# jbush001/RustNetworkStack

Measured on AMD Instinct MI355X. Metric: GiB/s device-resident Internet checksum, 1500B-packet batches, 1/2/4/8 GPUs, higher is better.
Workload: dtype u8

## Files before the change

rustnetworkstack_amd/csrc/k_packed.hip:

```cpp
#include "rns_launch.hpp"

#ifndef RNS_ROWS_DEEP_FROM
#define RNS_ROWS_DEEP_FROM 1024u
#endif
#ifndef RNS_TX_ROWS_DEEP_FROM
#define RNS_TX_ROWS_DEEP_FROM 1024u
#endif
#ifndef RNS_RX_ROWS_D
#define RNS_RX_ROWS_D 8
#endif

namespace rns {

constexpr bool kStreamNT = RNS_STREAM_NT != 0;

template <class Kernel>
static int launch_rows(const CsumArgs &a, uint32_t deep_from, hipStream_t st, Kernel kernel)
{
    return with_flags(
        [&](auto deep, auto buf) {
            return launch(kernel(std::integral_constant<int, deep() ? 16 : 8>{}, buf), dim3(waves64(a.n)), dim3(64), 0,
                          st, a);
        },
        a.len_hint >= deep_from, buf_ok(a));
}

int launch_stream_rx(const CsumArgs &a, hipStream_t st)
{
    return with_flags(
        [&](auto ack, auto buf) {
            if constexpr (ack())
                return launch(csum_stream_kernel<kStreamNT, buf()>, dim3(waves64(a.n)), dim3(64), 0, st, a);
            else
                return launch(csum_rows_rx_kernel<kStreamNT, buf(), RNS_RX_ROWS_D>, dim3(waves64(a.n)), dim3(64), 0, st,
                              a);
        },
        a.arena_bytes / a.n <= 128, buf_ok(a));
}

int dispatch_packed(const CsumArgs &a, const Shape &sh, hipStream_t st)
{
    const bool tiny = (sh.variant & ~16u) == 3u && sh.G == 4u && sh.U == 1u;
    if (a.align_mask >= 15u && !tiny)
        return launch_rows(a, RNS_ROWS_DEEP_FROM, st,
                           [](auto D, auto buf) { return csum_rows_kernel<kStreamNT, buf(), D()>; });
    const bool mixed = (sh.variant & 4u) != 0;
    if (!mixed && !tiny)
        return RNS_E_INVALID;
    const uint64_t batches = waves64(a.n);
    const uint64_t wpb = (mixed ? kMixedBlock<false> : kBlock) / 64;
    uint64_t blocks = (batches + wpb - 1) / wpb;
    if (sh.max_blocks != 0 && blocks > sh.max_blocks)
        blocks = sh.max_blocks;
    const dim3 grid(static_cast<uint32_t>(blocks)), block(mixed ? kMixedBlock<false> : kBlock);
    if (mixed)
        return with_flags(
            [&](auto nt, auto buf) {
                return launch(csum_mixed_kernel<false, nt(), buf(), false, false, false, true>, grid, block, 0, st, a);
            },
            (sh.variant & 2u) != 0, buf_ok(a));
    return with_flags(
        [&](auto buf, auto pf) {
            return launch(csum_rounds_kernel<4, 1, false, true, buf(), 1, true, pf()>, grid, block, 0, st, a);
        },
        buf_ok(a), (sh.variant & 16u) != 0);
}

int launch_fill_packed(const CsumArgs &a, hipStream_t st)
{
    return launch_rows(a, RNS_ROWS_DEEP_FROM, st,
                       [](auto D, auto buf) { return csum_rows_kernel<kStreamNT, buf(), D(), true>; });
}

int launch_tx_packed(const CsumArgs &a, hipStream_t st)
{
    return launch_rows(a, RNS_TX_ROWS_DEEP_FROM, st,
                       [](auto D, auto buf) { return csum_rows_tx_kernel<kStreamNT, buf(), D()>; });
}

int launch_strided_rx(const CsumArgs &a, hipStream_t st)
{
    constexpr int B = kStridedRxB;
    const dim3 grid(static_cast<uint32_t>((static_cast<uint64_t>(a.n) + 64 * B - 1) / (64 * B)));
    return with_flags([&](auto buf) { return launch(csum_strided_rx_kernel<buf(), B>, grid, dim3(64), 0, st, a); },
                      buf_ok(a));
}

}
```

rustnetworkstack_amd/csrc/rns_checksum.hip:

```cpp
#include <hip/hip_runtime.h>

#include <algorithm>
#include <cmath>
#include <cstdint>
#include <cstdio>

#include "rns_launch.hpp"

using namespace rns;

namespace {

__global__ __launch_bounds__(kBlock) void splitmix64_fill_kernel(uint8_t *buf, uint64_t nbytes, uint64_t seed)
{
    const uint64_t nwords = (nbytes + 7) / 8;
    const uint64_t stride = static_cast<uint64_t>(gridDim.x) * blockDim.x;
    for (uint64_t i = static_cast<uint64_t>(blockIdx.x) * blockDim.x + threadIdx.x; i < nwords; i += stride) {
        uint64_t z = seed + (i + 1) * 0x9E3779B97F4A7C15ull;
        z = (z ^ (z >> 30)) * 0xBF58476D1CE4E5B9ull;
        z = (z ^ (z >> 27)) * 0x94D049BB133111EBull;
        z = z ^ (z >> 31);
        if ((i + 1) * 8 <= nbytes) {
            reinterpret_cast<uint64_t *>(buf)[i] = z;
        } else {
// ... 69 lines not shown
}

void set_field(CsumArgs &a, const uint16_t *d_field, uint32_t field_off)
{
    a.field = d_field;
    a.field_off = field_off;
}

uint32_t be_sum(const uint8_t *p, int nbytes)
{
    uint32_t s = 0;
    for (int k = 0; k < nbytes; k += 2)
        s += static_cast<uint32_t>(p[k]) << 8 | p[k + 1];
    return s;
}

void set_rx(CsumArgs &a, uint8_t *d_status, uint16_t *d_l4_sum, const uint8_t *local_ipv4, const uint8_t *local_ipv6)
{
    a.status = d_status;
    a.l4_out = d_l4_sum;
    a.local4_sum = be_sum(local_ipv4, 4);
    a.local6_sum = be_sum(local_ipv6, 16);
}

bool rx_valid(const uint8_t *d_status, const uint8_t *local_ipv4, const uint8_t *local_ipv6)
{
    return d_status && local_ipv4 && local_ipv6;
}

void set_tx_status(CsumArgs &a, uint8_t *d_status) { a.status = d_status; }

uint32_t chain_pick_k(double mean)
{
    uint32_t K = 1;
    double best = -1.0;
    for (uint32_t k = 1; k <= kChainMaxK; ++k) {
        const double fr = k * mean, fill = fr > 0 ? fr / std::ceil(fr) : 1.0;
        if (fill > best + 0.02) {
            best = fill;
            K = k;
        }
    }
    return K;
}

double chain_mean(const CsumArgs &a) { return static_cast<double>(a.n_frags) / static_cast<double>(a.n); }

#ifndef RNS_CHAIN_NT_FROM
#define RNS_CHAIN_NT_FROM 384u
#endif
bool chain_nt_from_hint(uint32_t frag_len_hint) { return (frag_len_hint ? frag_len_hint : 512u) >= RNS_CHAIN_NT_FROM; }
bool chain_nt_from_arena(uint64_t arena_bytes, uint32_t n_frags, double mean)
{
    const double frag_est = mean > 0.5 ? static_cast<double>(arena_bytes) / n_frags * (mean - 0.5) / mean : 0.0;
    return n_frags == 0 || frag_est >= RNS_CHAIN_NT_FROM;
}

bool chain_deep(uint32_t K, double mean) { return K >= 3 || (K == 2 && mean >= 2.0); }

template <bool FILL>
int chain_launch(CsumArgs &a, uint32_t frag_len_hint, hipStream_t stream)
{
    const double mean = chain_mean(a);
    a.chain_k = chain_pick_k(mean);
    if ((a.flags & RNS_FLAG_CHAIN_TX_PACKED) && mean <= 1.0 + kRunFrags)
        return launch_txrows<FILL>(a, stream);
    const bool runs = kChainRuns && (a.flags & RNS_FLAG_CHAIN_RUNS) && buf_ok(a);
    return launch_chain<FILL>(a, a.chain_k, chain_nt_from_hint(frag_len_hint), runs, chain_deep(a.chain_k, mean), stream);
}

constexpr uint64_t kRxGridCap = 4096;
dim3 stash_grid(uint64_t n, uint64_t arena_bytes, bool tiny_cap)
{
    constexpr int BLK = kMixedBlock<true>;
    uint64_t blocks = (waves64(n) + BLK / 64 - 1) / (BLK / 64);
    const bool cap = tiny_cap && arena_bytes / n <= 128;
    if (cap && blocks > kRxGridCap)
        blocks = kRxGridCap;
    return dim3(static_cast<uint32_t>(blocks));
}

bool misaligned(const void *p, uintptr_t mask) { return (reinterpret_cast<uintptr_t>(p) & mask) != 0; }

bool pool_rx_valid(const uint8_t *d_pool, uint32_t buf_log2, uint32_t min_log2, const uint32_t *d_buf_idx, uint32_t n_frags,
                   const uint32_t *d_blk_first, const uint16_t *d_len16, uint32_t n_pkts, const uint8_t *local_ipv4,
                   const uint8_t *local_ipv6, const uint8_t *d_status)
{
    return d_pool && buf_log2 >= min_log2 && buf_log2 <= kPoolMaxLog2 && d_blk_first && d_len16 && (!n_frags || d_buf_idx) &&
           n_pkts <= RNS_CHAIN_MAX_PACKETS && !misaligned(d_pool, 15) && rx_valid(d_status, local_ipv4, local_ipv6);
}

int pool_rx_verify(PoolRx &rx, bool &nt, const uint8_t *d_pool, uint64_t pool_bytes, uint32_t buf_log2,
                   const uint32_t *d_buf_idx, uint32_t n_frags, const uint32_t *d_blk_first, const uint16_t *d_len16,
                   uint32_t n_pkts, const uint8_t *local_ipv4, const uint8_t *local_ipv6, uint8_t *d_status, uint16_t *d_l4_sum,
                   void *stream)
{
    RNS_TRY(rns_rx_verify_pool_dev(d_pool, pool_bytes, buf_log2, d_buf_idx, n_frags, d_blk_first, d_len16, n_pkts, local_ipv4,
                                   local_ipv6, d_status, d_l4_sum, stream));
    rx = PoolRx{d_pool, pool_bytes, d_buf_idx, d_blk_first, d_len16, d_status, n_pkts, n_frags, buf_log2};
    nt = chain_nt_from_arena(pool_bytes, n_frags, static_cast<double>(n_frags) / n_pkts);
    return RNS_OK;
}

bool pool_tx_valid(const uint8_t *d_tx_pool, const uint32_t *d_free, uint32_t n_free, uint32_t cap, const uint32_t *d_ip_id_add,
                   const uint32_t *d_tx_blk_first, const uint8_t *d_tx_head_len8, const uint16_t *d_tx_pay_len16,
                   const uint32_t *d_tx_src, const uint32_t *d_count)
{
    return d_tx_pool && d_count && (!n_free || d_free) && (!cap || (d_tx_blk_first && d_tx_head_len8 && d_tx_pay_len16)) &&
           !misaligned(d_tx_pool, 15) && !misaligned(d_free, 3) && !misaligned(d_ip_id_add, 3) &&
           !misaligned(d_tx_blk_first, 3) && !misaligned(d_tx_pay_len16, 1) && !misaligned(d_tx_src, 3) &&
           !misaligned(d_count, 3);
}

void set_pool_tx(PoolTx &tx, uint8_t *d_tx_pool, uint64_t tx_pool_bytes, uint32_t buf_log2, const uint32_t *d_free,
                 uint32_t n_free, uint32_t cap, uint16_t ip_id_base, const uint32_t *d_ip_id_add, uint32_t *d_tx_blk_first,
                 uint8_t *d_tx_head_len8, uint16_t *d_tx_pay_len16, uint32_t *d_tx_src, uint32_t *d_count)
{
    tx = PoolTx{d_tx_pool, tx_pool_bytes >> buf_log2, d_free, d_ip_id_add, d_tx_blk_first, d_tx_head_len8, d_tx_pay_len16,
                d_tx_src, d_count, n_free, cap, ip_id_base, buf_log2};
}

int count_only(uint32_t *d_count, size_t bytes, void *stream)
{
    if (!d_count || misaligned(d_count, 3))
        return RNS_E_INVALID;
    RNS_TRY(check_device());
    return launch_fill32(d_count, bytes / 4, 0u, static_cast<hipStream_t>(stream));
}

}

extern "C" {

int rns_csum_batch_dev_cfg(const uint8_t *d_arena, uint64_t arena_bytes, const uint64_t *d_off,
                           const uint32_t *d_len, const uint16_t *d_seed, uint16_t *d_out, uint32_t n,
                           uint32_t flags, uint32_t variant, uint32_t lanes_per_packet, uint32_t unroll,
                           uint32_t max_blocks, uint32_t *d_bad, void *stream)
{
    return entry(n, d_off && d_len && d_out, d_arena, arena_bytes, flags, stream, [&](CsumArgs &a, hipStream_t st) {
        set_explicit(a, d_off, d_len);
        set_results(a, d_seed, d_out, d_bad);
        return dispatch<false>(a, variant, lanes_per_packet, unroll, max_blocks, st);
    });
}

int rns_csum_batch_dev(const uint8_t *d_arena, uint64_t arena_bytes, const uint64_t *d_off,
                       const uint32_t *d_len, const uint16_t *d_seed, uint16_t *d_out, uint32_t n,
                       uint32_t flags, uint32_t len_hint, uint32_t *d_bad, void *stream)
{
    const Shape sh = pick_shape(len_hint);
    return rns_csum_batch_dev_cfg(d_arena, arena_bytes, d_off, d_len, d_seed, d_out, n, flags, sh.variant, sh.G,
                                  sh.U, sh.max_blocks, d_bad, stream);
}

int rns_csum_batch_dev_off32(const uint8_t *d_arena, uint64_t arena_bytes, const uint32_t *d_off32,
                             const uint32_t *d_len, const uint16_t *d_seed, uint16_t *d_out, uint32_t n,
                             uint32_t flags, uint32_t len_hint, uint32_t *d_bad, void *stream)
{
    return entry(n, d_off32 && d_len && d_out, d_arena, arena_bytes, flags, stream, [&](CsumArgs &a, hipStream_t st) {
        a.off32 = d_off32;
        a.len = d_len;
        set_results(a, d_seed, d_out, d_bad);
        const Shape sh = pick_shape(len_hint);
        return dispatch<false>(a, sh.variant, sh.G, sh.U, sh.max_blocks, st);
    });
}

int rns_csum_batch_packed_dev(const uint8_t *d_arena, uint64_t arena_bytes, const uint64_t *d_blk_off,
                              const uint16_t *d_len16, uint32_t align_log2, const uint16_t *d_seed, uint16_t *d_out,
                              uint32_t n, uint32_t flags, uint32_t len_hint, uint32_t *d_bad, void *stream)
{
    return entry(n, d_blk_off && d_len16 && d_out && packed_align(align_log2, 0), d_arena, arena_bytes, flags, stream,
                 [&](CsumArgs &a, hipStream_t st) {
                     set_packed(a, d_blk_off, d_len16, align_log2);
                     set_results(a, d_seed, d_out, d_bad);
                     a.len_hint = len_hint;
                     Shape sh = pick_shape(len_hint);
                     if ((sh.variant & 5u) == 0)
                         sh = Shape{6u, 0u, 0u, 0u};
                     return dispatch_packed(a, sh, st);
                 });
}

int rns_csum_batch_strided_dev(const uint8_t *d_arena, uint64_t arena_bytes, uint64_t first_off,
                               uint64_t stride, uint32_t len, const uint16_t *d_seed, uint16_t *d_out,
                               uint32_t n, uint32_t flags, uint32_t *d_bad, void *stream)
{
    return entry(n, d_out && strided_fits(first_off, stride, n), d_arena, arena_bytes, flags, stream,
                 [&](CsumArgs &a, hipStream_t st) {
                     set_strided(a, first_off, stride);
                     set_results(a, d_seed, d_out, d_bad);
                     a.fixed_len = len;
                     if (len != 0 && len <= 64 && ((first_off + a.base_adjust) & 15) == 0 && (stride & 15) == 0)
                         return launch_strided_tiny(a, st);
                     const Shape sh = pick_shape(len);
                     return dispatch<true>(a, sh.variant, sh.G, sh.U, sh.max_blocks, st);
                 });
}

int rns_csum_chain_dev(const uint8_t *d_arena, uint64_t arena_bytes, const uint64_t *d_frag_off,
                       const uint32_t *d_frag_len, uint32_t n_frags, const uint32_t *d_first,
                       const uint16_t *d_seed, uint16_t *d_out, uint32_t n_pkts, uint32_t flags,
                       uint32_t frag_len_hint, uint16_t *d_frag_sums, uint32_t *d_bad, void *stream)
{
    (void)d_frag_sums;
    return entry(n_pkts, d_out && chain_valid(d_frag_off, d_frag_len, d_first, n_frags, n_pkts), d_arena, arena_bytes,
                 flags, stream, [&](CsumArgs &a, hipStream_t st) {
                     set_chain(a, d_frag_off, d_frag_len, d_first, n_frags);
                     set_results(a, d_seed, d_out, d_bad);
                     return chain_launch<false>(a, frag_len_hint, st);
                 });
}

int rns_csum_chain_fill_dev(uint8_t *d_arena, uint64_t arena_bytes, const uint64_t *d_frag_off,
                            const uint32_t *d_frag_len, uint32_t n_frags, const uint32_t *d_first,
                            const uint16_t *d_seed, const uint16_t *d_field, uint32_t field_off, uint16_t *d_out,
                            uint32_t n_pkts, uint32_t flags, uint32_t frag_len_hint, uint32_t *d_bad, void *stream)
{
    return entry(n_pkts, chain_valid(d_frag_off, d_frag_len, d_first, n_frags, n_pkts), d_arena, arena_bytes, flags,
                 stream, [&](CsumArgs &a, hipStream_t st) {
                     set_chain(a, d_frag_off, d_frag_len, d_first, n_frags);
                     set_results(a, d_seed, d_out, d_bad);
                     set_field(a, d_field, field_off);
                     return chain_launch<true>(a, frag_len_hint, st);
                 });
}

int rns_csum_fill_dev(uint8_t *d_arena, uint64_t arena_bytes, const uint64_t *d_off, const uint32_t *d_len,
                      const uint16_t *d_seed, const uint16_t *d_field, uint32_t field_off, uint16_t *d_out,
                      uint32_t n, uint32_t flags, uint32_t *d_bad, void *stream)
{
    return entry(n, d_off && d_len, d_arena, arena_bytes, flags, stream, [&](CsumArgs &a, hipStream_t st) {
        set_explicit(a, d_off, d_len);
        set_results(a, d_seed, d_out, d_bad);
        set_field(a, d_field, field_off);
        return launch_fill(a, stash_grid(n, arena_bytes, false), st);
    });
}

int rns_csum_fill_packed_dev(uint8_t *d_arena, uint64_t arena_bytes, const uint64_t *d_blk_off, const uint16_t *d_len16,
                             uint32_t align_log2, const uint16_t *d_seed, const uint16_t *d_field, uint32_t field_off,
                             uint16_t *d_out, uint32_t n, uint32_t flags, uint32_t len_hint, uint32_t *d_bad,
                             void *stream)
{
    return entry(n, d_blk_off && d_len16 && packed_align(align_log2, 4), d_arena, arena_bytes, flags, stream,
                 [&](CsumArgs &a, hipStream_t st) {
                     set_packed(a, d_blk_off, d_len16, align_log2);
                     set_results(a, d_seed, d_out, d_bad);
                     set_field(a, d_field, field_off);
                     a.len_hint = len_hint;
                     return launch_fill_packed(a, st);
                 });
}

int rns_rx_verify_dev(const uint8_t *d_arena, uint64_t arena_bytes, const uint64_t *d_off, const uint32_t *d_len,
                      uint32_t n, const uint8_t *local_ipv4, const uint8_t *local_ipv6, uint8_t *d_status,
                      uint16_t *d_l4_sum, void *stream)
{
    return entry(n, d_off && d_len && rx_valid(d_status, local_ipv4, local_ipv6), d_arena, arena_bytes,
                 RNS_FLAG_COMPLEMENT, stream, [&](CsumArgs &a, hipStream_t st) {
                     set_explicit(a, d_off, d_len);
                     set_rx(a, d_status, d_l4_sum, local_ipv4, local_ipv6);
                     return launch_rx(a, stash_grid(n, arena_bytes, true), st);
                 });
}

int rns_rx_verify_packed_dev(const uint8_t *d_arena, uint64_t arena_bytes, const uint64_t *d_blk_off,
                             const uint16_t *d_len16, uint32_t align_log2, uint32_t n, const uint8_t *local_ipv4,
                             const uint8_t *local_ipv6, uint8_t *d_status, uint16_t *d_l4_sum, void *stream)
{
    return entry(n, d_blk_off && d_len16 && rx_valid(d_status, local_ipv4, local_ipv6) && packed_align(align_log2, 4),
                 d_arena, arena_bytes, RNS_FLAG_COMPLEMENT, stream, [&](CsumArgs &a, hipStream_t st) {
                     set_packed(a, d_blk_off, d_len16, align_log2);
                     set_rx(a, d_status, d_l4_sum, local_ipv4, local_ipv6);
                     return launch_stream_rx(a, st);
                 });
}

int rns_rx_verify_strided_dev(const uint8_t *d_arena, uint64_t arena_bytes, uint64_t first_off, uint64_t stride,
                              const uint16_t *d_len16, uint32_t n, const uint8_t *local_ipv4, const uint8_t *local_ipv6,
                              uint8_t *d_status, uint16_t *d_l4_sum, void *stream)
{
    return entry(n, d_len16 && rx_valid(d_status, local_ipv4, local_ipv6) && strided_fits(first_off, stride, n), d_arena,
                 arena_bytes, RNS_FLAG_COMPLEMENT, stream, [&](CsumArgs &a, hipStream_t st) {
                     a.len16 = d_len16;
                     set_strided(a, first_off, stride);
                     set_rx(a, d_status, d_l4_sum, local_ipv4, local_ipv6);
                     return launch_strided_rx(a, st);
                 });
}

int rns_rx_verify_chain_dev(const uint8_t *d_arena, uint64_t arena_bytes, const uint64_t *d_frag_off,
                            const uint32_t *d_frag_len, uint32_t n_frags, const uint32_t *d_first, uint32_t n_pkts,
                            const uint8_t *local_ipv4, const uint8_t *local_ipv6, uint8_t *d_status, uint16_t *d_l4_sum,
                            void *stream)
{
    return entry(n_pkts,
                 chain_valid(d_frag_off, d_frag_len, d_first, n_frags, n_pkts) &&
                     rx_valid(d_status, local_ipv4, local_ipv6),
                 d_arena, arena_bytes, RNS_FLAG_COMPLEMENT, stream, [&](CsumArgs &a, hipStream_t st) {
                     set_chain(a, d_frag_off, d_frag_len, d_first, n_frags);
                     set_rx(a, d_status, d_l4_sum, local_ipv4, local_ipv6);
                     const double mean = chain_mean(a);
                     a.chain_k = chain_pick_k(mean);
                     return launch_rx_chain(a, a.chain_k, chain_nt_from_arena(arena_bytes, n_frags, mean), st);
                 });
}

int rns_rx_verify_pool_dev(const uint8_t *d_pool, uint64_t pool_bytes, uint32_t buf_log2, const uint32_t *d_buf_idx,
                           uint32_t n_frags, const uint32_t *d_blk_first, const uint16_t *d_len16, uint32_t n_pkts,
                           const uint8_t *local_ipv4, const uint8_t *local_ipv6, uint8_t *d_status, uint16_t *d_l4_sum,
                           void *stream)
{
    return entry(n_pkts,
                 pool_rx_valid(d_pool, buf_log2, kPoolMinLog2, d_buf_idx, n_frags, d_blk_first, d_len16, n_pkts, local_ipv4,
                               local_ipv6, d_status),
                 d_pool, pool_bytes, RNS_FLAG_COMPLEMENT, stream, [&](CsumArgs &a, hipStream_t st) {
                     a.off32 = d_buf_idx;
                     a.n_frags = n_frags;
                     a.first = d_blk_first;
                     a.len16 = d_len16;
                     a.align_mask = (1u << buf_log2) - 1u;
                     set_rx(a, d_status, d_l4_sum, local_ipv4, local_ipv6);
                     const double mean = chain_mean(a);
                     a.chain_k = chain_pick_k(mean);
                     return launch_rx_pool(a, a.chain_k, chain_nt_from_arena(pool_bytes, n_frags, mean), st);
                 });
}

int rns_rx_tcp_place_pool_dev(const uint8_t *d_pool, uint64_t pool_bytes, uint32_t buf_log2, const uint32_t *d_buf_idx,
                              uint32_t n_frags, const uint32_t *d_blk_first, const uint16_t *d_len16, uint32_t n_pkts,
                              const uint8_t *local_ipv4, const uint8_t *local_ipv6, const uint8_t *d_tbl,
                              uint64_t tbl_bytes, const uint32_t *d_next_seq, const uint64_t *d_win_off,
                              const uint32_t *d_win_len, uint32_t n_flows, uint8_t *d_stream, uint64_t stream_bytes,
                              uint8_t *d_status, uint16_t *d_l4_sum, rns_rx_tcp_meta *d_meta, void *stream)
{
    static_assert(sizeof(rns_rx_tcp_meta) == 24 && sizeof(rns_rx_flow_key) == kFlowSlotBytes - 8, "rns_k_pool_place.hpp");
    if (n_pkts == 0)
        return RNS_OK;
    const uint64_t slots = flow_slots(n_flows);
    if (!pool_rx_valid(d_pool, buf_log2, kPlaceMinLog2, d_buf_idx, n_frags, d_blk_first, d_len16, n_pkts, local_ipv4,
                       local_ipv6, d_status) ||
        !d_meta || misaligned(d_meta, 3) || !d_next_seq || !d_win_off || !d_win_len || !d_stream ||
        (n_flows && (!d_tbl || misaligned(d_tbl, 3) || tbl_bytes < slots * kFlowSlotBytes)))
        return RNS_E_INVALID;
    PoolRx rx;
// ... 382 lines not shown
                     set_tx_status(a, d_status);
                     return launch_txrows<false, true, true>(a, st);
                 });
}

int rns_tx_fill_pool_dev(uint8_t *d_pool, uint64_t pool_bytes, uint32_t buf_log2, const uint32_t *d_buf_idx,
                         uint32_t n_frags, const uint32_t *d_blk_first, const uint8_t *d_head_len8,
                         const uint16_t *d_pay_len16, uint32_t n_pkts, uint8_t *d_status, void *stream)
{
    return entry(n_pkts,
                 buf_log2 >= kPoolTxMinLog2 && buf_log2 <= kPoolMaxLog2 && d_blk_first && d_head_len8 && d_pay_len16 &&
                     (!n_frags || d_buf_idx) && n_pkts <= RNS_CHAIN_MAX_PACKETS &&
                     (reinterpret_cast<uintptr_t>(d_pool) & 15) == 0,
                 d_pool, pool_bytes, RNS_FLAG_COMPLEMENT, stream, [&](CsumArgs &a, hipStream_t st) {
                     a.off32 = d_buf_idx;
                     a.n_frags = n_frags;
                     a.first = d_blk_first;
                     a.head_len8 = d_head_len8;
                     a.len16 = d_pay_len16;
                     a.align_mask = (1u << buf_log2) - 1u;
                     set_tx_status(a, d_status);
                     const double mean = chain_mean(a);
                     a.chain_k = chain_pick_k(mean);
                     return launch_tx_pool(a, a.chain_k, chain_nt_from_arena(pool_bytes, n_frags, mean), st);
                 });
}

int rns_tx_segment_dev(uint8_t *d_arena, uint64_t arena_bytes, const uint8_t *d_tmpl, uint32_t tmpl_stride,
                       const uint8_t *d_head_len8, const uint64_t *d_pay_off, const uint32_t *d_pay_len,
                       const uint16_t *d_mss, const uint64_t *d_head_off, const uint32_t *d_seg_first,
                       const uint32_t *d_blk_flow, uint32_t n_flows, uint32_t n_seg, uint8_t *d_status, void *stream)
{
    return entry(n_flows ? n_seg : 0u,
                 d_tmpl && tmpl_stride && d_head_len8 && d_pay_off && d_pay_len && d_mss && d_head_off && d_seg_first &&
                     d_blk_flow && n_seg <= RNS_CHAIN_MAX_PACKETS,
                 d_arena, arena_bytes, RNS_FLAG_COMPLEMENT, stream, [&](CsumArgs &a, hipStream_t st) {
                     a.tmpl = d_tmpl;
                     a.tmpl_stride = tmpl_stride;
                     a.n_flows = n_flows;
                     a.head_len8 = d_head_len8;
                     a.seg_pay_off = d_pay_off;
                     a.len = d_pay_len;
                     a.len16 = d_mss;
                     a.seg_head_off = d_head_off;
                     a.first = d_seg_first;
                     a.blk_flow = d_blk_flow;
                     set_tx_status(a, d_status);
                     return launch_tx_segment(a, arena_bytes / n_seg >= RNS_CHAIN_NT_FROM, st);
                 });
}

int rns_tx_fill_dev(uint8_t *d_arena, uint64_t arena_bytes, const uint64_t *d_off, const uint32_t *d_len,
                    uint32_t n, uint8_t *d_status, void *stream)
{
    return entry(n, d_off && d_len, d_arena, arena_bytes, RNS_FLAG_COMPLEMENT, stream, [&](CsumArgs &a, hipStream_t st) {
        set_explicit(a, d_off, d_len);
        set_tx_status(a, d_status);
        return launch_tx(a, stash_grid(n, arena_bytes, true), st);
    });
}

int rns_fill_splitmix64_dev(uint8_t *d_buf, uint64_t nbytes, uint64_t seed, void *stream)
{
    if (nbytes == 0)
        return RNS_OK;
    if (!d_buf || (reinterpret_cast<uintptr_t>(d_buf) & 7))
        return RNS_E_INVALID;
    RNS_TRY(check_device());
    const uint64_t words = (nbytes + 7) / 8;
    const uint32_t blocks = static_cast<uint32_t>(std::min<uint64_t>((words + kBlock - 1) / kBlock, 8192));
    hipLaunchKernelGGL(splitmix64_fill_kernel, dim3(blocks), dim3(kBlock), 0, static_cast<hipStream_t>(stream),
                       d_buf, nbytes, seed);
    return hip_status(hipGetLastError());
}

const char *rns_csum_shape_name(uint32_t len_hint)
{
    static const char *const names[] = {"csum_batch_kernel",     "csum_rounds_kernel",     "csum_batch_kernel[nt]",
                                        "csum_rounds_kernel[nt]", "csum_mixed_kernel",      "csum_mixed_kernel",
                                        "csum_mixed_kernel[nt]",  "csum_mixed_kernel[nt]"};
    static thread_local char buf[96];
    const Shape sh = pick_shape(len_hint);
    if (sh.variant & 4)
        std::snprintf(buf, sizeof(buf), "%s (size classes G/U 4/1 x 4 packets, 4/4, 16/4, 32/4, 64/4)", names[sh.variant & 7]);
    else
        std::snprintf(buf, sizeof(buf), "%s<G=%u,U=%u>%s%s", names[sh.variant & 7], sh.G, sh.U,
                      (sh.variant & 8) ? " all rounds in flight" : (sh.variant & 16) ? " descriptors prefetched" : "",
                      sh.max_blocks ? " grid-capped" : "");
    return buf;
}

const char *rns_build_info(void)
{
    return "rns_checksum abi=1 offload-arch=gfx950 kernels=csum_rows_kernel (packed form: 1 KiB rows per 64-packet "
           "region, owners capture two region prefixes and sum their own end chunk; fill mode), csum_rows_rx_kernel "
           "(packed receive verify: the rows plus each owner's header chunks loaded a group ahead), csum_stream_kernel "
           "(receive verify of ACK-sized arenas: owners load their datagrams whole), csum_strided_rx_kernel (receive "
           "verify of fixed-size slots: quad-coalesced rows), csum_rows_tx_kernel (packed transmit finalize through the "
           "rows), csum_txrows_kernel (transmit-shaped chains: packed payload rows + owner-loaded head fragments; "
           "head-fragment fill; whole finalize of NetBuffer chains with the heads written back from LDS), "
           "csum_strided_tiny_kernel "
           "(fixed-size packets <= 64 B at a fixed stride), csum_mixed_kernel (per-wave size-class sort; verify / fill / "
           "transmit-finalize stash modes), csum_rounds_kernel, csum_batch_kernel, csum_chain_kernel (one pass, "
           "per-fragment fold; head-fragment fill) (v_sad_u16 LE sums, v_dot4 BE sums past 128 KiB, wave64, DPP "
           "reductions)";
}

int rns_device_count(void)
{
    int n = 0;
    if (hipGetDeviceCount(&n) != hipSuccess) {
        (void)hipGetLastError();
        return 0;
    }
    return n;
}

}
```

rustnetworkstack_amd/csrc/rns_kernels.hpp:

```cpp
#pragma once

#include "rns_k_tcp_head.hpp"
#include "rns_k_common.hpp"
#include "rns_k_rounds.hpp"
#include "rns_k_mixed.hpp"
#include "rns_k_chain.hpp"
#include "rns_k_chain_rx.hpp"
#include "rns_k_pool_rx.hpp"
#include "rns_k_stream.hpp"
#include "rns_k_rows.hpp"
#include "rns_k_rows_rx.hpp"
#include "rns_k_rows_tx.hpp"
#include "rns_k_txrows.hpp"
#include "rns_k_pool_tx.hpp"
#include "rns_k_segment.hpp"
#include "rns_k_pool_view.hpp"
#include "rns_k_pool_place.hpp"
#include "rns_k_scan.hpp"
#include "rns_k_pool_txform.hpp"
#include "rns_k_args.hpp"
```

rustnetworkstack_amd/csrc/rns_launch.hpp:

```cpp
#pragma once

#include <type_traits>

#include "rns_kernels.hpp"

namespace rns {

inline int hip_status(hipError_t e) { return e == hipSuccess ? RNS_OK : RNS_E_HIP_BASE - static_cast<int>(e); }

struct Shape {
    uint32_t variant, G, U, max_blocks;
};

constexpr uint32_t kTinyVariant = 19u;
constexpr uint32_t kTinyGrid = 2048u;
inline Shape pick_shape(uint32_t len_hint)
{
    const uint32_t chunks = len_hint ? (len_hint + 15) / 16 + 1 : 96;
    if (chunks <= 8)
        return Shape{kTinyVariant, 4u, 1u, kTinyGrid};
    if (chunks <= 48)
        return Shape{4u, 0u, 0u, 0u};
    if (chunks <= 160)
        return Shape{6u, 0u, 0u, 0u};
    return Shape{2u, 64u, 4u, 0u};
}

inline int check_device()
{
    int n = 0;
    if (hipGetDeviceCount(&n) != hipSuccess || n <= 0) {
        (void)hipGetLastError();
        return RNS_E_NODEVICE;
    }
    return RNS_OK;
}

inline void set_arena(CsumArgs &a, const uint8_t *arena, uint64_t arena_bytes)
{
    const uintptr_t p = reinterpret_cast<uintptr_t>(arena);
    a.base_adjust = p & 15;
    a.arena = reinterpret_cast<const uint8_t *>(p - a.base_adjust);
    a.arena_bytes = arena_bytes + a.base_adjust;
}

inline bool buf_ok(const CsumArgs &a) { return buf_records(a) < kOobOffset; }

inline uint32_t waves64(uint64_t n) { return static_cast<uint32_t>((n + 63) / 64); }

template <class F>
int with_flags(F &&f)
{
    return f();
}
template <class F, class... Rest>
int with_flags(F &&f, bool b, Rest... rest)
{
    auto bind = [&](auto c) { return with_flags([&](auto... cs) { return f(c, cs...); }, rest...); };
    return b ? bind(std::true_type{}) : bind(std::false_type{});
}

template <uint32_t KM, uint32_t... More, class F>
int with_kmax(uint32_t K, F &&f)
{
    if constexpr (sizeof...(More) == 0)
        return f(std::integral_constant<uint32_t, KM>{});
    else
        return K <= KM ? f(std::integral_constant<uint32_t, KM>{}) : with_kmax<More...>(K, f);
}

inline int launch(void (*kernel)(const CsumArgs), dim3 grid, dim3 block, size_t lds, hipStream_t st, const CsumArgs &a)
{
    hipLaunchKernelGGL(kernel, grid, block, lds, st, a);
    return hip_status(hipGetLastError());
}

#define RNS_TRY(status)          \
    do {                         \
        if (int e = (status))    \
            return e;            \
    } while (0)
#define RNS_LAUNCH(kernel, grid, block, st, ...)                                      \
    do {                                                                              \
        hipLaunchKernelGGL(kernel, dim3(grid), dim3(block), 0, st, __VA_ARGS__);      \
        RNS_TRY(hip_status(hipGetLastError()));                                       \
    } while (0)

int launch_scan2_parts(uint2 *part, uint32_t nb, uint32_t *total2, hipStream_t st);
int launch_fill32(uint32_t *p, uint64_t n, uint32_t v, hipStream_t st);

template <class Classify, class Build>
int launch_build_seq(uint32_t *count, const BuildWork &w, uint64_t n, hipStream_t st, Classify classify, Build build)
{
    const uint32_t nb = static_cast<uint32_t>(scan_blocks(n));
    RNS_TRY(launch_fill32(count, 3, 0u, st));
    RNS_TRY(classify(nb));
    RNS_TRY(launch_scan2_parts(w.part_a, nb, nullptr, st));
    RNS_TRY(launch_scan2_parts(w.part_b, nb, nullptr, st));
    return build(nb);
}

template <bool S>
int dispatch(const CsumArgs &a, uint32_t variant, uint32_t G, uint32_t U, uint32_t max_blocks, hipStream_t st);
extern template int dispatch<false>(const CsumArgs &, uint32_t, uint32_t, uint32_t, uint32_t, hipStream_t);
extern template int dispatch<true>(const CsumArgs &, uint32_t, uint32_t, uint32_t, uint32_t, hipStream_t);
int launch_strided_tiny(const CsumArgs &a, hipStream_t st);
int dispatch_packed(const CsumArgs &a, const Shape &sh, hipStream_t st);
int launch_fill_packed(const CsumArgs &a, hipStream_t st);
int launch_stream_rx(const CsumArgs &a, hipStream_t st);
int launch_tx_packed(const CsumArgs &a, hipStream_t st);
int launch_strided_rx(const CsumArgs &a, hipStream_t st);
template <bool FILL>
int launch_chain(const CsumArgs &a, uint32_t K, bool nt, bool runs, bool deep, hipStream_t st);
extern template int launch_chain<false>(const CsumArgs &, uint32_t, bool, bool, bool, hipStream_t);
extern template int launch_chain<true>(const CsumArgs &, uint32_t, bool, bool, bool, hipStream_t);
template <bool FILL, bool FIN = false, bool CPT = false>
int launch_txrows(const CsumArgs &a, hipStream_t st);
extern template int launch_txrows<false, false, false>(const CsumArgs &, hipStream_t);
extern template int launch_txrows<true, false, false>(const CsumArgs &, hipStream_t);
extern template int launch_txrows<false, true, false>(const CsumArgs &, hipStream_t);
extern template int launch_txrows<false, true, true>(const CsumArgs &, hipStream_t);
int launch_rx_chain(const CsumArgs &a, uint32_t K, bool nt, hipStream_t st);
int launch_rx_pool(const CsumArgs &a, uint32_t K, bool nt, hipStream_t st);
int launch_tx_pool(const CsumArgs &a, uint32_t K, bool nt, hipStream_t st);
int launch_tx_segment(const CsumArgs &a, bool nt, hipStream_t st);
int launch_rx_place(const PlaceArgs &a, bool nt, hipStream_t st);
int launch_flow_update(const FlowArgs &a, hipStream_t st);
int launch_ack_build(const AckArgs &a, hipStream_t st);
int launch_flow_lists(const FlowArgs &a, uint32_t rec_dw, hipStream_t st);
int launch_conn_update(const FlowArgs &a, hipStream_t st);
int launch_ctl_build(const CtlArgs &a, hipStream_t st);
int launch_conn_close(const CloseArgs &a, hipStream_t st);
int launch_tx_plan(const PlanArgs &a, hipStream_t st);
int launch_rx_echo(const EchoArgs &a, bool nt, hipStream_t st);
int launch_rx_udp(const UdpArgs &a, bool nt, hipStream_t st);
int launch_tx_udp(const UdpTxArgs &a, hipStream_t st);
int launch_rx_listen(const ListenArgs &a, hipStream_t st);
int launch_fill(const CsumArgs &a, dim3 grid, hipStream_t st);
int launch_rx(const CsumArgs &a, dim3 grid, hipStream_t st);
int launch_tx(const CsumArgs &a, dim3 grid, hipStream_t st);

}
```

rustnetworkstack_amd/csrc/rns_k_rows.hpp:

```cpp
#pragma once

#include "rns_k_stream.hpp"

namespace rns {

#ifndef RNS_ROWS_FILL_OCC
#define RNS_ROWS_FILL_OCC 6
#endif
#ifndef RNS_ROWS_FILL_BLOCK
#define RNS_ROWS_FILL_BLOCK 32
#endif
template <bool NT, bool BUF, int D, bool FILL = false>
__global__ __launch_bounds__(64, D >= 16 ? 4 : FILL ? RNS_ROWS_FILL_OCC : 8) void csum_rows_kernel(const CsumArgs a)
{
    const uint32_t lane = threadIdx.x;
    const __amdgpu_buffer_rsrc_t rsrc = __builtin_amdgcn_make_buffer_rsrc(
        const_cast<uint8_t *>(a.arena), static_cast<short>(0), static_cast<int>(BUF ? buf_records(a) : 0), 0x00020000);
    const uint64_t recs = buf_records(a);
    const PackedUnit u = packed_unit(a, lane);
    const uint64_t p = u.p, q = u.q, r0 = u.r0, start = u.start();
    const uint32_t len = u.len, excl = u.excl, total = u.total;
    const uint32_t seed = u.seed;
    const bool live = u.live, ok = u.ok(a);
    constexpr uint32_t FB = FILL ? RNS_ROWS_FILL_BLOCK : 16u, FC = FB / 16u;
    uint32_t fo = 0;
    if constexpr (FILL)
        fo = a.field ? static_cast<uint32_t>(a.field[q]) : a.field_off;
    const bool fok = FILL && live && ok && fo <= len && len - fo >= 2u;
    const uint64_t fpos = start + fo, fch = fpos & ~15ull;
    const uint32_t back = ((static_cast<uint32_t>(reinterpret_cast<uintptr_t>(a.arena) >> 4) +
                            static_cast<uint32_t>(fch >> 4)) & (FC - 1u)) * 16u;
    const uint64_t sec = fch - back;
    const bool sec_ok = fok && fch >= back && sec + FB <= recs;
    const uint32_t rel = static_cast<uint32_t>(fpos - sec);
    uint4 sv[FC];
    uint32_t fb0 = 0, fb1 = 0;
    if constexpr (FILL) {
#pragma unroll
        for (uint32_t i = 0; i < FC; ++i) {
            if constexpr (BUF) {
                const uint32_t o = sec_ok ? static_cast<uint32_t>(sec) + 16u * i : kOobOffset;
                const u32x4 x = __builtin_amdgcn_raw_buffer_load_b128(rsrc, o, 0, 0);
                sv[i] = make_uint4(x.x, x.y, x.z, x.w);
            } else {
                sv[i] = sec_ok ? load_chunk<false>(a.arena + sec + 16u * i) : make_uint4(0, 0, 0, 0);
            }
        }
        if (fok && (!sec_ok || rel == FB - 1u)) {
            fb0 = a.arena[fpos];
            fb1 = a.arena[fpos + 1];
        }
        __builtin_amdgcn_sched_barrier(0);
    }
    uint32_t mine = 0;
    bool odd = false;
    if ((r0 & 15) == 0) {
        const uint32_t c0 = excl >> 4;
        const uint32_t e = len ? (excl + len - 1) >> 4 : c0;
        mine = rows_region_sum<NT, BUF, D>(a, rsrc, recs, r0, total, c0, e, len);
    } else {
        const uint64_t start = r0 + excl;
        const bool ok = start <= a.arena_bytes && len <= a.arena_bytes - start;
        uint64_t todo = __ballot(len != 0 && ok);
        while (todo) {
            const uint32_t o = static_cast<uint32_t>(__builtin_ctzll(todo));
            todo &= todo - 1;
            const uint64_t st =
                (static_cast<uint64_t>(static_cast<uint32_t>(__builtin_amdgcn_readlane(static_cast<uint32_t>(start >> 32), o)))
                 << 32) |
                static_cast<uint32_t>(__builtin_amdgcn_readlane(static_cast<uint32_t>(start), o));
            const uint32_t L = __builtin_amdgcn_readlane(len, o);
            const Pkt k = make_pkt(st, L);
            uint32_t acc = 0;
            for (uint32_t cc = 0; cc < k.nch; cc += 64) {
                uint4 w[1];
                issue_pass<64, 1, NT, BUF, 1>(a, rsrc, k, cc + lane, w);
                mask_edges<64, 1, 1>(k, cc + lane, w);
                acc = sum_le<1, 1>(w, acc);
            }
            const uint32_t sum = group_allreduce<64>(acc);
            mine = lane == o ? sum : mine;
        }
        odd = r0 & 1;
    }
    if constexpr (FILL) {
        uint32_t w[4 * FC];
#pragma unroll
        for (uint32_t i = 0; i < FC; ++i) {
            w[4 * i] = sv[i].x;
            w[4 * i + 1] = sv[i].y;
            w[4 * i + 2] = sv[i].z;
            w[4 * i + 3] = sv[i].w;
        }
        uint32_t b0 = fb0, b1 = fb1;
        if (sec_ok && rel != FB - 1u) {
            uint32_t d0 = 0, d1 = 0;
#pragma unroll
            for (uint32_t d = 0; d < 4 * FC; ++d) {
                d0 = (rel >> 2) == d ? w[d] : d0;
                d1 = ((rel + 1u) >> 2) == d ? w[d] : d1;
            }
            b0 = (d0 >> ((rel & 3u) * 8u)) & 0xffu;
// ... 108 lines not shown
```

rustnetworkstack_amd/csrc/rns_k_stream.hpp:

```cpp
#pragma once

#include "rns_k_chain.hpp"

namespace rns {

__device__ __forceinline__ uint4 keep_first(uint4 v, uint32_t c)
{
    const uint32_t bits = c * 8u;
    const uint64_t lo = ~0ull >> (64u - min(bits, 64u));
    const uint64_t hi = bits > 64u ? ~0ull >> ((128u - bits) & 63u) : 0ull;
    v.x &= static_cast<uint32_t>(lo);
    v.y &= static_cast<uint32_t>(lo >> 32);
    v.z &= static_cast<uint32_t>(hi);
    v.w &= static_cast<uint32_t>(hi >> 32);
    return v;
}

#ifndef RNS_STREAM_NT
#define RNS_STREAM_NT 1
#endif
#ifndef RNS_STREAM_OUT_AUX
#define RNS_STREAM_OUT_AUX 17
#endif
constexpr int kStreamD = 8;
constexpr int kStreamRxOcc = 6;

template <bool BUF>
__device__ __forceinline__ uint4 own_chunk(const CsumArgs &a, __amdgpu_buffer_rsrc_t rsrc, uint64_t recs, uint64_t off,
                                           uint32_t len, uint32_t i)
{
    const uint64_t o = off + 16u * i;
    return load16<BUF, false>(a, rsrc, o, 16u * i < len && o + 16 <= recs);
}

__device__ __forceinline__ void store_rx_status(const CsumArgs &a, uint64_t p, uint8_t stv, uint32_t l4_res)
{
    a.status[p] = stv;
    if (a.l4_out)
        a.l4_out[p] = static_cast<uint16_t>(l4_res);
}

template <bool NT, bool BUF>
__device__ __forceinline__ void wave_serial_sums(const CsumArgs &a, __amdgpu_buffer_rsrc_t rsrc, uint32_t lane,
                                                 uint64_t todo, uint64_t start, uint32_t len, uint32_t &mine)
{
    while (todo) {
        const uint32_t o = static_cast<uint32_t>(__builtin_ctzll(todo));
        todo &= todo - 1;
        const Pkt k = make_pkt(lane_u64(start, o), __builtin_amdgcn_readlane(len, o));
        uint32_t acc = 0;
        for (uint32_t cc = 0; cc < k.nch; cc += 64) {
            uint4 w[1];
            issue_pass<64, 1, NT, BUF, 1>(a, rsrc, k, cc + lane, w);
            mask_edges<64, 1, 1>(k, cc + lane, w);
            acc = sum_le<1, 1>(w, acc);
        }
        const uint32_t sum = group_allreduce<64>(acc);
        mine = lane == o ? sum : mine;
    }
}

struct PackedUnit {
    uint64_t p, q;
    bool live;
    uint32_t len, seed;
    uint64_t r0;
    uint32_t excl, total;
    __device__ __forceinline__ uint64_t start() const { return r0 + excl; }
    __device__ __forceinline__ bool ok(const CsumArgs &a) const
    {
        return start() <= a.arena_bytes && len <= a.arena_bytes - start();
    }
};

__device__ __forceinline__ PackedUnit packed_unit(const CsumArgs &a, uint32_t lane)
{
    PackedUnit u;
    const uint64_t base = static_cast<uint64_t>(blockIdx.x) * 64;
    u.p = base + lane;
    u.live = u.p < a.n;
    u.q = u.live ? u.p : a.n - 1;
    const uint32_t zero_v = __builtin_amdgcn_mbcnt_lo(0u, 0u);
    const uint64_t r0v = a.blk_off[(base >> 6) + zero_v];
    u.len = u.live ? static_cast<uint32_t>(a.len16[u.q]) : 0u;
    u.seed = (a.seed && u.live) ? static_cast<uint32_t>(a.seed[u.q]) : 0u;
    u.r0 = first_lane_u64(r0v) + a.base_adjust;
    const uint32_t pad = (u.len + a.align_mask) & ~a.align_mask;
    const uint32_t incl = wave_incl_scan(pad);
    u.excl = incl - pad;
    u.total = __builtin_amdgcn_readlane(incl, 63);
    return u;
}

template <bool BUF, bool MASKED, int N>
__device__ __forceinline__ uint32_t ack_unit_sum(const CsumArgs &a, __amdgpu_buffer_rsrc_t rsrc, uint64_t recs,
                                                 uint64_t start, uint32_t len, uint4 (&own)[N])
{
    static_assert(N >= 4, "four chunks hold an ACK-sized packet");
    uint32_t mine = 0;
#pragma unroll
    for (int i = 0; i < 4; ++i)
        own[i] = own_chunk<BUF>(a, rsrc, recs, start, len, i);
#pragma unroll
    for (int i = 0; i < 4; ++i) {
        uint4 x = own[i];
        if (16u * i + 16u > len)
            x = 16u * i < len ? keep_first(x, len - 16u * i) : make_uint4(0, 0, 0, 0);
        if constexpr (MASKED)
            own[i] = x;
        mine = sad4(x, mine);
    }
    return mine;
}

template <bool BUF, int N>
__device__ __forceinline__ uint32_t unaligned_head(const CsumArgs &a, __amdgpu_buffer_rsrc_t rsrc, uint64_t recs,
                                                   uint64_t start, uint32_t len, bool present, uint4 (&own)[N])
{
    const uint64_t b0 = start & ~15ull;
    const uint32_t s0 = static_cast<uint32_t>(start & 15);
#pragma unroll
    for (int i = 0; i < N; ++i)
        own[i] = own_chunk<BUF>(a, rsrc, recs, b0, present ? s0 + len : 0u, i);
#pragma unroll
    for (int i = 0; i < N; ++i) {
        const int lo = static_cast<int>(s0) - 16 * i, hi = static_cast<int>(s0 + len) - 16 * i;
        own[i] = make_uint4(keep_bytes(own[i].x, lo, hi, 0), keep_bytes(own[i].y, lo, hi, 4),
                            keep_bytes(own[i].z, lo, hi, 8), keep_bytes(own[i].w, lo, hi, 12));
    }
    return s0;
}

template <bool NT, bool BUF>
__global__ __launch_bounds__(64, kStreamRxOcc) void csum_stream_kernel(const CsumArgs a)
{
    constexpr int kNS = 4;
    constexpr uint32_t kTagShift = 17, kHead = 1u << 16, kEnd = 1u << 13, kStart = 1u << 12;
    __shared__ uint32_t tab[64];
    __shared__ uint32_t pend[64];
    __shared__ uint32_t pstart[64];
    __shared__ uint4 stash[64 * kNS];
    const uint32_t lane = threadIdx.x;
    const __amdgpu_buffer_rsrc_t rsrc = __builtin_amdgcn_make_buffer_rsrc(
        const_cast<uint8_t *>(a.arena), static_cast<short>(0), static_cast<int>(BUF ? buf_records(a) : 0), 0x00020000);
    const uint64_t recs = buf_records(a);
    const PackedUnit u = packed_unit(a, lane);
    const uint64_t p = u.p, r0 = u.r0;
    const uint32_t len = u.len, excl = u.excl, total = u.total;
    const bool live = u.live;
    uint32_t mine = 0;
    bool odd = false;

    if ((r0 & 15) == 0 && !__ballot(len > 64)) {
        const uint64_t start = u.start();
        const bool ok = u.ok(a);
        uint4 own[kNS + 1];
        mine = ack_unit_sum<BUF, true>(a, rsrc, recs, start, len, own);
        own[4] = make_uint4(0, 0, 0, 0);
        uint32_t l4_res = 0;
// ... 205 lines not shown
```

Baseline: 6729.

## Route explicit-descriptor checksums through per-wave row tiling when descriptors tile

```diff
diff --git a/rustnetworkstack_amd/csrc/k_packed.hip b/rustnetworkstack_amd/csrc/k_packed.hip
--- a/rustnetworkstack_amd/csrc/k_packed.hip
+++ b/rustnetworkstack_amd/csrc/k_packed.hip
@@ -1,8 +1,5 @@
 #include "rns_launch.hpp"
 
-#ifndef RNS_ROWS_DEEP_FROM
-#define RNS_ROWS_DEEP_FROM 1024u
-#endif
 #ifndef RNS_TX_ROWS_DEEP_FROM
 #define RNS_TX_ROWS_DEEP_FROM 1024u
 #endif
diff --git a/rustnetworkstack_amd/csrc/k_rows_explicit.hip b/rustnetworkstack_amd/csrc/k_rows_explicit.hip
--- /dev/null
+++ b/rustnetworkstack_amd/csrc/k_rows_explicit.hip
@@ -0,0 +1,24 @@
+#include "rns_launch.hpp"
+
+namespace rns {
+
+int launch_rows_explicit(const CsumArgs &a, bool nt, bool deep, hipStream_t st)
+{
+    return with_flags(
+        [&](auto NT, auto DEEP, auto BUF) {
+            return launch(csum_rows_explicit_kernel<NT(), BUF(), DEEP() ? 16 : 8>, dim3(waves64(a.n)), dim3(64), 0, st, a);
+        },
+        nt, deep, buf_ok(a));
+}
+
+int launch_rows_explicit_rx(const CsumArgs &a, bool deep, hipStream_t st)
+{
+    return with_flags(
+        [&](auto DEEP, auto BUF) {
+            return launch(csum_rows_explicit_rx_kernel<true, BUF(), DEEP() ? 16 : 8>, dim3(waves64(a.n)), dim3(64), 0, st,
+                          a);
+        },
+        deep, buf_ok(a));
+}
+
+}
diff --git a/rustnetworkstack_amd/csrc/rns_checksum.hip b/rustnetworkstack_amd/csrc/rns_checksum.hip
--- a/rustnetworkstack_amd/csrc/rns_checksum.hip
+++ b/rustnetworkstack_amd/csrc/rns_checksum.hip
@@ -175,6 +175,14 @@
 
 bool misaligned(const void *p, uintptr_t mask) { return (reinterpret_cast<uintptr_t>(p) & mask) != 0; }
 
+int dispatch_explicit(const CsumArgs &a, uint32_t len_hint, hipStream_t st)
+{
+    const Shape sh = pick_shape(len_hint);
+    if (sh.variant & 4u)
+        return launch_rows_explicit(a, (sh.variant & 2u) != 0, len_hint >= RNS_ROWS_DEEP_FROM, st);
+    return dispatch<false>(a, sh.variant, sh.G, sh.U, sh.max_blocks, st);
+}
+
 bool pool_rx_valid(const uint8_t *d_pool, uint32_t buf_log2, uint32_t min_log2, const uint32_t *d_buf_idx, uint32_t n_frags,
                    const uint32_t *d_blk_first, const uint16_t *d_len16, uint32_t n_pkts, const uint8_t *local_ipv4,
                    const uint8_t *local_ipv6, const uint8_t *d_status)
@@ -241,9 +249,11 @@
                        const uint32_t *d_len, const uint16_t *d_seed, uint16_t *d_out, uint32_t n,
                        uint32_t flags, uint32_t len_hint, uint32_t *d_bad, void *stream)
 {
-    const Shape sh = pick_shape(len_hint);
-    return rns_csum_batch_dev_cfg(d_arena, arena_bytes, d_off, d_len, d_seed, d_out, n, flags, sh.variant, sh.G,
-                                  sh.U, sh.max_blocks, d_bad, stream);
+    return entry(n, d_off && d_len && d_out, d_arena, arena_bytes, flags, stream, [&](CsumArgs &a, hipStream_t st) {
+        set_explicit(a, d_off, d_len);
+        set_results(a, d_seed, d_out, d_bad);
+        return dispatch_explicit(a, len_hint, st);
+    });
 }
 
 int rns_csum_batch_dev_off32(const uint8_t *d_arena, uint64_t arena_bytes, const uint32_t *d_off32,
@@ -254,8 +264,7 @@
         a.off32 = d_off32;
         a.len = d_len;
         set_results(a, d_seed, d_out, d_bad);
-        const Shape sh = pick_shape(len_hint);
-        return dispatch<false>(a, sh.variant, sh.G, sh.U, sh.max_blocks, st);
+        return dispatch_explicit(a, len_hint, st);
     });
 }
 
@@ -354,7 +363,9 @@
                  RNS_FLAG_COMPLEMENT, stream, [&](CsumArgs &a, hipStream_t st) {
                      set_explicit(a, d_off, d_len);
                      set_rx(a, d_status, d_l4_sum, local_ipv4, local_ipv6);
-                     return launch_rx(a, stash_grid(n, arena_bytes, true), st);
+                     if (arena_bytes / n <= 128)
+                         return launch_rx(a, stash_grid(n, arena_bytes, true), st);
+                     return launch_rows_explicit_rx(a, arena_bytes / n >= RNS_ROWS_DEEP_FROM, st);
                  });
 }
 
@@ -903,7 +914,8 @@
     static thread_local char buf[96];
     const Shape sh = pick_shape(len_hint);
     if (sh.variant & 4)
-        std::snprintf(buf, sizeof(buf), "%s (size classes G/U 4/1 x 4 packets, 4/4, 16/4, 32/4, 64/4)", names[sh.variant & 7]);
+        std::snprintf(buf, sizeof(buf), "csum_rows_explicit_kernel<D=%d>%s (rows per tiling wave, else size classes)",
+                      len_hint >= RNS_ROWS_DEEP_FROM ? 16 : 8, (sh.variant & 2) ? "[nt]" : "");
     else
         std::snprintf(buf, sizeof(buf), "%s<G=%u,U=%u>%s%s", names[sh.variant & 7], sh.G, sh.U,
                       (sh.variant & 8) ? " all rounds in flight" : (sh.variant & 16) ? " descriptors prefetched" : "",
@@ -915,7 +927,9 @@
 {
     return "rns_checksum abi=1 offload-arch=gfx950 kernels=csum_rows_kernel (packed form: 1 KiB rows per 64-packet "
            "region, owners capture two region prefixes and sum their own end chunk; fill mode), csum_rows_rx_kernel "
-           "(packed receive verify: the rows plus each owner's header chunks loaded a group ahead), csum_stream_kernel "
+           "(packed receive verify: the rows plus each owner's header chunks loaded a group ahead), "
+           "csum_rows_explicit_kernel / csum_rows_explicit_rx_kernel (explicit descriptors: the rows for each wave whose "
+           "64 descriptors tile, else the class pass), csum_stream_kernel "
            "(receive verify of ACK-sized arenas: owners load their datagrams whole), csum_strided_rx_kernel (receive "
            "verify of fixed-size slots: quad-coalesced rows), csum_rows_tx_kernel (packed transmit finalize through the "
            "rows), csum_txrows_kernel (transmit-shaped chains: packed payload rows + owner-loaded head fragments; "
diff --git a/rustnetworkstack_amd/csrc/rns_k_rows_explicit.hpp b/rustnetworkstack_amd/csrc/rns_k_rows_explicit.hpp
--- /dev/null
+++ b/rustnetworkstack_amd/csrc/rns_k_rows_explicit.hpp
@@ -0,0 +1,122 @@
+#pragma once
+
+#include "rns_k_rows_rx.hpp"
+
+namespace rns {
+
+struct ExplicitWave {
+    uint64_t p;
+    bool live, ok;
+    uint64_t start;
+    uint32_t len;
+    uint32_t seed;
+    bool tiles;
+    uint64_t r0;
+    uint32_t span, c0, e;
+};
+
+constexpr bool kRowsExplicitNT = RNS_STREAM_NT != 0;
+
+template <bool BUF>
+__device__ __forceinline__ ExplicitWave explicit_wave(const CsumArgs &a, uint32_t lane)
+{
+    ExplicitWave w;
+    w.p = static_cast<uint64_t>(blockIdx.x) * 64 + lane;
+    w.live = w.p < a.n;
+    const Desc<BUF> cd = load_desc<false, false, BUF>(a, w.p);
+    w.start = cd.off + a.base_adjust;
+    w.len = cd.len;
+    w.seed = (a.seed && w.live) ? a.seed[w.p] : 0u;
+    w.ok = w.start <= a.arena_bytes && w.len <= a.arena_bytes - w.start;
+    if (!w.ok || w.len == 0) {
+        w.len = 0;
+        w.start = 0;
+    }
+    const bool present = w.len != 0;
+    const uint32_t s_lo = static_cast<uint32_t>(w.start), s_hi = static_cast<uint32_t>(w.start >> 32);
+    uint32_t r_hi = 0;
+    if constexpr (!BUF)
+        r_hi = wave_min_u32(present ? s_hi : 0xFFFFFFFFu);
+    const uint32_t r_lo = wave_min_u32(present && s_hi == r_hi ? s_lo : 0xFFFFFFFFu);
+    w.r0 = (static_cast<uint64_t>(r_hi) << 32) | r_lo;
+    const uint64_t rel64 = w.start - w.r0;
+    const bool fits = (w.start & 15) == 0 && w.len <= 0xFFFFu && rel64 < (1ull << 26);
+    const uint32_t rel = static_cast<uint32_t>(rel64);
+    const uint32_t pad = present && fits ? (w.len + 15u) & ~15u : 0u;
+    w.span = wave_max_u32(pad ? rel + pad : 0u);
+    const uint32_t sum_pad = __builtin_amdgcn_readlane(wave_incl_scan(pad), 63);
+    w.tiles = __ballot(present) && !__ballot(present && !fits) && w.span <= 2u * sum_pad + 4096u;
+    w.c0 = pad ? rel >> 4 : 0u;
+    w.e = pad ? (rel + w.len - 1u) >> 4 : 0u;
+    return w;
+}
+
+template <bool NT, bool BUF, int D>
+__global__ __launch_bounds__(64, (D >= 16 || !BUF) ? 4 : 5) void csum_rows_explicit_kernel(const CsumArgs a)
+{
+    const uint32_t lane = threadIdx.x;
+    const __amdgpu_buffer_rsrc_t rsrc = __builtin_amdgcn_make_buffer_rsrc(
+        const_cast<uint8_t *>(a.arena), static_cast<short>(0), static_cast<int>(BUF ? buf_records(a) : 0), 0x00020000);
+    const uint64_t recs = buf_records(a);
+    const ExplicitWave w = explicit_wave<BUF>(a, lane);
+    const bool odd = w.start & 1, big = w.len > kNoWrapBytes;
+    uint32_t mine;
+    if (w.tiles) {
+        mine = rows_region_sum<kRowsExplicitNT, BUF, D>(a, rsrc, recs, w.r0, w.span, w.c0, w.e, w.len);
+    } else {
+        uint32_t pos;
+        mine = wave_class_pass<NT, BUF, kStashNone>(a, rsrc, w.start, w.len, 0xFFFFFFFFu, lane, nullptr, pos);
+    }
+    const uint16_t res = finalize_bits(mine, odd, big, w.seed, w.ok, a.flags);
+    uint32_t lane2 = threadIdx.x;
+    asm volatile("" : "+v"(lane2));
+    const uint64_t p = static_cast<uint64_t>(blockIdx.x) * 64 + lane2;
+    if (w.live && a.out)
+        __builtin_nontemporal_store(res, a.out + p);
+    count_rejected(a, lane, w.live && !w.ok);
+}
+
+template <bool NT, bool BUF, int D>
+__global__ __launch_bounds__(64, RNS_STASH_OCC) void csum_rows_explicit_rx_kernel(const CsumArgs a)
+{
+    constexpr int kNS = kStashChunks<kStashHead>;
+    __shared__ uint4 stash_lds[64 * kNS];
+    const uint32_t lane = threadIdx.x;
+    const __amdgpu_buffer_rsrc_t rsrc = __builtin_amdgcn_make_buffer_rsrc(
+        const_cast<uint8_t *>(a.arena), static_cast<short>(0), static_cast<int>(BUF ? buf_records(a) : 0), 0x00020000);
+    const uint64_t recs = buf_records(a);
+    const ExplicitWave w = explicit_wave<BUF>(a, lane);
+    const bool present = w.live && w.len != 0;
+    uint32_t l4_res = 0;
+    uint8_t stv;
+    if (w.tiles) {
+        constexpr int kNH = 4;
+        uint4 own[kNH + 1];
+        own[kNH] = make_uint4(0, 0, 0, 0);
+        const uint32_t mine =
+            rows_region_sum<kRowsExplicitNT, BUF, D, 3>(a, rsrc, recs, w.r0, w.span, w.c0, w.e, w.len, own);
+        {
+            const uint32_t b0 = own[0].x & 0xffu;
+            const bool need = present && w.len > 48 && (b0 >> 4) == 4 && (b0 & 15u) > 12;
+            if (__ballot(need))
+                own[3] = need ? own_chunk<BUF>(a, rsrc, recs, w.start, w.len, 3) : make_uint4(0, 0, 0, 0);
+            else
+                own[3] = make_uint4(0, 0, 0, 0);
+        }
+#pragma unroll
+        for (int i = 0; i < kNH; ++i)
+            if (16u * i + 16u > w.len)
+                own[i] = 16u * i < w.len ? keep_first(own[i], w.len - 16u * i) : make_uint4(0, 0, 0, 0);
+        stv = rx_finish<kNH + 1>(a, own, mine, 0u, w.len, false, false, present, l4_res);
+    } else {
+        uint32_t pos;
+        const uint32_t mine = wave_class_pass<NT, BUF, kStashHead>(a, rsrc, w.start, w.len, 0xFFFFFFFFu, lane, stash_lds, pos);
+        wave_lds_fence();
+        stv = rx_finish<kNS>(a, stash_lds + pos * kNS, mine, static_cast<uint32_t>(w.start & 15), w.len, w.start & 1,
+                             w.len > kNoWrapBytes, present, l4_res);
+    }
+    if (w.live)
+        store_rx_status(a, w.p, stv, l4_res);
+}
+
+}
diff --git a/rustnetworkstack_amd/csrc/rns_kernels.hpp b/rustnetworkstack_amd/csrc/rns_kernels.hpp
--- a/rustnetworkstack_amd/csrc/rns_kernels.hpp
+++ b/rustnetworkstack_amd/csrc/rns_kernels.hpp
@@ -10,6 +10,7 @@
 #include "rns_k_stream.hpp"
 #include "rns_k_rows.hpp"
 #include "rns_k_rows_rx.hpp"
+#include "rns_k_rows_explicit.hpp"
 #include "rns_k_rows_tx.hpp"
 #include "rns_k_txrows.hpp"
 #include "rns_k_pool_tx.hpp"
diff --git a/rustnetworkstack_amd/csrc/rns_launch.hpp b/rustnetworkstack_amd/csrc/rns_launch.hpp
--- a/rustnetworkstack_amd/csrc/rns_launch.hpp
+++ b/rustnetworkstack_amd/csrc/rns_launch.hpp
@@ -25,6 +25,10 @@
         return Shape{6u, 0u, 0u, 0u};
     return Shape{2u, 64u, 4u, 0u};
 }
+
+#ifndef RNS_ROWS_DEEP_FROM
+#define RNS_ROWS_DEEP_FROM 1024u
+#endif
 
 inline int check_device()
 {
@@ -110,6 +114,8 @@
 int launch_stream_rx(const CsumArgs &a, hipStream_t st);
 int launch_tx_packed(const CsumArgs &a, hipStream_t st);
 int launch_strided_rx(const CsumArgs &a, hipStream_t st);
+int launch_rows_explicit(const CsumArgs &a, bool nt, bool deep, hipStream_t st);
+int launch_rows_explicit_rx(const CsumArgs &a, bool deep, hipStream_t st);
 template <bool FILL>
 int launch_chain(const CsumArgs &a, uint32_t K, bool nt, bool runs, bool deep, hipStream_t st);
 extern template int launch_chain<false>(const CsumArgs &, uint32_t, bool, bool, bool, hipStream_t);
```

Result: no change. 6724 (-0.1%).

## Split 64-packet row blocks into 4-packet sub-units for long packets

Applied to the files above, without the earlier changes.

```diff
diff --git a/rustnetworkstack_amd/csrc/k_packed.hip b/rustnetworkstack_amd/csrc/k_packed.hip
--- a/rustnetworkstack_amd/csrc/k_packed.hip
+++ b/rustnetworkstack_amd/csrc/k_packed.hip
@@ -25,6 +25,29 @@
         a.len_hint >= deep_from, buf_ok(a));
 }
 
+constexpr uint32_t kSubTarget = 40u << 10;
+static uint32_t rows_sub_unit(uint32_t len_hint)
+{
+    const uint64_t padded = (static_cast<uint64_t>(len_hint) + 15u) & ~15ull;
+    return 8 * padded > kSubTarget ? 4u : 64u;
+}
+
+static int launch_rows_csum(const CsumArgs &a, hipStream_t st)
+{
+    constexpr uint32_t S = 4;
+    static_assert(kSubTarget / 8 >= RNS_ROWS_DEEP_FROM, "every hint that takes sub-units takes D = 16");
+    if (rows_sub_unit(a.len_hint) == 64)
+        return launch_rows(a, RNS_ROWS_DEEP_FROM, st,
+                           [](auto D, auto buf) { return csum_rows_kernel<kStreamNT, buf(), D()>; });
+    const uint64_t grid = (static_cast<uint64_t>(waves64(a.n)) + 7) / 8 * 8 * (64u / S);
+    return with_flags(
+        [&](auto buf) {
+            return launch(csum_rows_kernel<kStreamNT, buf(), 16, false, static_cast<int>(S)>,
+                          dim3(static_cast<uint32_t>(grid)), dim3(64), 0, st, a);
+        },
+        buf_ok(a));
+}
+
 int launch_stream_rx(const CsumArgs &a, hipStream_t st)
 {
     return with_flags(
@@ -42,8 +65,7 @@
 {
     const bool tiny = (sh.variant & ~16u) == 3u && sh.G == 4u && sh.U == 1u;
     if (a.align_mask >= 15u && !tiny)
-        return launch_rows(a, RNS_ROWS_DEEP_FROM, st,
-                           [](auto D, auto buf) { return csum_rows_kernel<kStreamNT, buf(), D()>; });
+        return launch_rows_csum(a, st);
     const bool mixed = (sh.variant & 4u) != 0;
     if (!mixed && !tiny)
         return RNS_E_INVALID;
diff --git a/rustnetworkstack_amd/csrc/rns_k_rows.hpp b/rustnetworkstack_amd/csrc/rns_k_rows.hpp
--- a/rustnetworkstack_amd/csrc/rns_k_rows.hpp
+++ b/rustnetworkstack_amd/csrc/rns_k_rows.hpp
@@ -10,14 +10,19 @@
 #ifndef RNS_ROWS_FILL_BLOCK
 #define RNS_ROWS_FILL_BLOCK 32
 #endif
-template <bool NT, bool BUF, int D, bool FILL = false>
+template <bool NT, bool BUF, int D, bool FILL = false, int S = 64>
 __global__ __launch_bounds__(64, D >= 16 ? 4 : FILL ? RNS_ROWS_FILL_OCC : 8) void csum_rows_kernel(const CsumArgs a)
 {
+    static_assert(!FILL || S == 64, "the fill form takes whole blocks");
     const uint32_t lane = threadIdx.x;
+    if constexpr (S != 64) {
+        if (sub_first<S>(blockIdx.x) >= a.n)
+            return;
+    }
     const __amdgpu_buffer_rsrc_t rsrc = __builtin_amdgcn_make_buffer_rsrc(
         const_cast<uint8_t *>(a.arena), static_cast<short>(0), static_cast<int>(BUF ? buf_records(a) : 0), 0x00020000);
     const uint64_t recs = buf_records(a);
-    const PackedUnit u = packed_unit(a, lane);
+    const PackedUnit u = packed_unit<S>(a, lane);
     const uint64_t p = u.p, q = u.q, r0 = u.r0, start = u.start();
     const uint32_t len = u.len, excl = u.excl, total = u.total;
     const uint32_t seed = u.seed;
diff --git a/rustnetworkstack_amd/csrc/rns_k_stream.hpp b/rustnetworkstack_amd/csrc/rns_k_stream.hpp
--- a/rustnetworkstack_amd/csrc/rns_k_stream.hpp
+++ b/rustnetworkstack_amd/csrc/rns_k_stream.hpp
@@ -73,8 +73,46 @@
     }
 };
 
+template <int S>
+__device__ __forceinline__ uint64_t sub_first(uint64_t b)
+{
+    constexpr uint64_t K = 64 / S;
+    const uint64_t g = b / (8 * K), r = b % (8 * K);
+    return (8 * g + (r & 7)) * 64 + (r >> 3) * S;
+}
+
+template <int S>
+__device__ __forceinline__ PackedUnit packed_sub_unit(const CsumArgs &a, uint32_t lane)
+{
+    static_assert(S == 32 || S == 16 || S == 8 || S == 4, "a sub-unit is a power-of-two part of a 64-packet block");
+    PackedUnit u;
+    const uint64_t first = sub_first<S>(blockIdx.x);
+    const uint64_t base = first & ~63ull;
+    const uint32_t rot = static_cast<uint32_t>(first) & 63u;
+    const uint64_t pb = base + ((rot + lane) & 63u);
+    const bool in = pb < a.n;
+    u.p = first + lane;
+    u.live = lane < static_cast<uint32_t>(S) && in;
+    u.q = u.live ? u.p : a.n - 1;
+    const uint32_t zero_v = __builtin_amdgcn_mbcnt_lo(0u, 0u);
+    const uint64_t r0v = a.blk_off[(base >> 6) + zero_v];
+    const uint32_t blen = in ? static_cast<uint32_t>(a.len16[in ? pb : a.n - 1]) : 0u;
+    u.len = u.live ? blen : 0u;
+    u.seed = (a.seed && u.live) ? static_cast<uint32_t>(a.seed[u.q]) : 0u;
+    const uint32_t pad = (blen + a.align_mask) & ~a.align_mask;
+    const uint32_t incl = wave_incl_scan(pad);
+    u.excl = incl - pad;
+    u.total = __builtin_amdgcn_readlane(incl, S - 1);
+    const uint32_t before = __builtin_amdgcn_readlane(incl, 63) - __builtin_amdgcn_readlane(incl, 63u - rot);
+    u.r0 = first_lane_u64(r0v) + a.base_adjust + before;
+    return u;
+}
+
+template <int S = 64>
 __device__ __forceinline__ PackedUnit packed_unit(const CsumArgs &a, uint32_t lane)
 {
+    if constexpr (S != 64)
+        return packed_sub_unit<S>(a, lane);
     PackedUnit u;
     const uint64_t base = static_cast<uint64_t>(blockIdx.x) * 64;
     u.p = base + lane;
```

Result: no change. 6723 before, 6708 after (-0.2%).
